# mikhaildubov/AST-text-analysis

Hardware: NVIDIA B200
Metric: keyphrase_x_doc_scores_per_sec (higher is better)
Workload: dtype f64

## Files before the change

### ast-text-analysis_b200/csrc/capi.cu

```cuda
#include <algorithm>
#include <array>
#include <chrono>
#include <cstdio>
#include <cstdlib>
#include <cstring>
#include <exception>
#include <map>
#include <memory>
#include <mutex>
#include <string>

#include "../../include/east_b200.h"
#include "sa_build.h"
#include "kp_prep.h"

namespace east {

thread_local int64_t g_launches = 0;
thread_local int g_time_kernels = 0;
thread_local double g_next_bytes = 0.0;

struct KernelStat { int64_t launches = 0; double ms = 0.0; double bytes = 0.0; };
struct PendingLaunch { std::string name; cudaEvent_t a, b; double bytes; };
static thread_local std::map<std::string, KernelStat> g_kstats;
// ... 474 lines not shown
    idx->next = take32((size_t)n);
    idx->ann = take32((size_t)n);

    if (text8_dev && !chunks) {
        DevBuf<uint32_t> bad(1, s);
        EAST_CUDA(cudaMemsetAsync(bad.p, 0, sizeof(uint32_t), s));
        expand_text8(text8_dev, idx->d_doc_off, idx->d_doc_m, n_docs, idx->text, bad.p, s);
        uint32_t h_bad = 0;
        EAST_CUDA(cudaMemcpyAsync(&h_bad, bad.p, sizeof(uint32_t), cudaMemcpyDeviceToHost, s));
        EAST_CUDA(cudaStreamSynchronize(s));
        if (h_bad) throw Error(EAST_ERR_INVALID, "one-byte text: a document does not hold exactly doc_m string ends (0xFF) or does not end with one");
    }
    idx->build_timer.reset(new StageTimer(s));
    StageTimer &tm = *idx->build_timer;
    const bool overlap = get_option("sync_build", 0) == 0;
    {
        SaInput in;
        in.text = idx->text; in.doc_off = idx->d_doc_off; in.doc_m = idx->d_doc_m;
        in.n = n; in.n_docs = n_docs; in.m_total = idx->m_total;
        in.key_chars = (int)get_option("key_chars", 0);
        in.force_general = (int)get_option("force_general", 0);
        in.rs_variant = (int)get_option("rs_variant", 0);
        in.doc_off_host = idx->doc_off.data();
        in.sort_batch_elems = get_option("sort_batch_elems", 0);
        in.local_group_sort = get_option("doubling_radix", 0) ? 0 : 1;
        in.segmented_sort = get_option("global_sort", 0) ? 0 : 1;
        in.doc_sort = (get_option("no_doc_sort", 0) || in.key_chars || in.rs_variant || in.sort_batch_elems ||
                       !in.segmented_sort || !in.local_group_sort) ? 0 : 1;
        in.want_bkt3 = get_option("no_bkt3", 0) ? 0 : 1;
        in.light_scan = get_option("no_light_scan", 0) ? 0 : 1;
        { const int64_t smp = get_option("alphabet_sample", (int64_t)1 << 21); in.alphabet_sample = smp < 0 ? 0 : smp; }
        in.alphabet_guess = get_option("no_alphabet_guess", 0) ? 0 : 1;
        in.fused_encode = get_option("no_fused_encode", 0) ? 0 : 1;
        if (!get_option("no_suffix_keys", 0)) {
            idx->sk = (uint32_t *)take32((size_t)n);
            in.sk = idx->sk;
        }
        if (!get_option("no_fused_tables", 0)) {
            in.lcp = idx->lcp; in.up = idx->up; in.down = idx->down; in.next = idx->next; in.ann = idx->ann;
        }
        in.arena = idx->arena.base ? &idx->arena : nullptr;
        in.helper_stream = aux_stream(device);
        if (!get_option("no_prep_stream", 0)) in.prep_stream = prep_stream(device);
        if (hook && hook->fn) {
            in.run_begin = hook->begin; in.run_hook = hook->fn; in.run_ctx = hook->ctx; in.scan_queued = hook->scan_queued;
            if (hook->building) *hook->building = idx.get();
        }
        if (chunks && text8_dev) {
            if (!in.doc_sort || !in.fused_encode) throw Error(EAST_ERR_INVALID, "internal: the one-byte pipelined build needs the per-document kernel");
            in.text8 = text8_dev;
        }
        if (chunks && in.doc_sort) {
            in.n_chunks = (int)chunks->ready.size();
            in.chunk_doc = chunks->doc.data();
            in.chunk_ready = chunks->ready.data();
        } else if (chunks) {
            for (auto e : chunks->ready) EAST_CUDA(cudaStreamWaitEvent(s, e, 0));
        }
        SaOutput so;
        so.sa = idx->sa;
        build_suffix_array(in, so, tm, s);
        idx->pipelined = so.pipelined; idx->pipeline_miss = so.pipeline_miss; idx->alphabet_miss = so.alphabet_miss; idx->alphabet_guessed = so.alphabet_guessed;
        idx->rounds = so.rounds; idx->fast_path = so.fast_path; idx->key_chars = so.key_chars;
        idx->key_bits = so.key_bits; idx->active_after_round0 = so.active_after_round0;
        idx->doc_sorted = so.doc_sorted; idx->doc_sort_overflow = so.doc_sort_overflow;
        idx->t8 = so.t8.p; so.t8.p = nullptr;
// ... 1216 lines not shown
```

### ast-text-analysis_b200/csrc/doc_sort.cu

```cuda
#include <cstdlib>
#include "sa_build.h"
#include "score_walk.cuh"

namespace east {

constexpr int DS_THREADS = 1024;
constexpr int DS_WARPS = DS_THREADS / 32;
constexpr int DS_GROUP = 128;
constexpr int DS_GWARPS = DS_GROUP / 32;
constexpr int DS_NGROUPS = DS_THREADS / DS_GROUP;
constexpr int DS_REFINE_MAX = 4096;
constexpr int DS_SUB_BINS = 1024;
constexpr int DS_GRP_BYTES = DS_REFINE_MAX * 2 + DS_SUB_BINS * 4;
constexpr int DS_SCR_BYTES = DS_NGROUPS * DS_GRP_BYTES;
constexpr int DS_WARP_MAX = 1024;
constexpr int DS_WARP_BYTES = DS_WARP_MAX * 2 + 128 * 4;
constexpr int DS_LIST_CAP = 2048;
constexpr int DS_WIN_BYTES = 64 * 8 + 64 * 4;
constexpr int DS_INF = 0x7fffffff;
static_assert(DS_WARPS * DS_WARP_BYTES <= DS_SCR_BYTES && DS_WARPS * DS_WIN_BYTES <= DS_SCR_BYTES, "scratch");
static_assert(8 * DocScore::MAX_GROUPS <= DS_SCR_BYTES, "phase 9 keeps the groups' maxima in shared memory");

struct DocSortParams {
    const uint8_t *t8;
    const uint32_t *text;
    const int32_t *doc_off;
    const int32_t *doc_m;
    int32_t *sa;
    uint32_t *bkt;
    uint32_t *bkt3;
    uint32_t *overflow;
    int b, G, S2;
    uint32_t term;
    int text_cap;
    int bits_words;
    int doc_begin;
    unsigned long long *phase_clk;
    int32_t *lcp, *up, *down, *next, *ann;
    uint32_t *sk;
    DocScore score;
    const uint8_t *code_table;
    uint8_t *t8_out;
    uint32_t *miss;
    int64_t text_len;
    const uint8_t *text8;
    uint32_t *text_out;
    int fill_early;
};

__device__ __forceinline__ uint64_t ds_lds8(const uint8_t *base, int o) {
    const uint32_t *q = reinterpret_cast<const uint32_t *>(base + (o & ~3));
    const uint32_t sh = (uint32_t)(o & 3) * 8u;
    const uint32_t w0 = q[0], w1 = q[1], w2 = q[2];
    return ((uint64_t)__funnelshift_r(w1, w2, sh) << 32) | __funnelshift_r(w0, w1, sh);
}
__device__ __forceinline__ uint32_t ds_lds4(const uint8_t *base, int o) {
    const uint32_t *q = reinterpret_cast<const uint32_t *>(base + (o & ~3));
    return __funnelshift_r(q[0], q[1], (uint32_t)(o & 3) * 8u);
}

__device__ __forceinline__ uint32_t ds_zero4(uint32_t v) {
    return ~(((v & 0x7f7f7f7fu) + 0x7f7f7f7fu) | v | 0x7f7f7f7fu);
}

__device__ __forceinline__ uint64_t ds_haszero(uint64_t v) {
    return (v - 0x0101010101010101ull) & ~v & 0x8080808080808080ull;
}

__device__ __forceinline__ uint32_t ds_id_from_word(uint32_t w, uint32_t term4, int b, int nsym) {
    const uint32_t z = ds_zero4(w ^ term4) & (0xffffffffu >> (8 * (4 - nsym)));
    if (z) w &= 0xffffffffu >> (8 * (3 - ((__ffs(z) - 1) >> 3)));
    const uint32_t s0 = w & 0xffu, s1 = (w >> 8) & 0xffu, s2 = (w >> 16) & 0xffu, s3 = w >> 24;
    switch (nsym) {
        case 1: return s0;
        case 2: return (s0 << b) | s1;
        case 3: return (((s0 << b) | s1) << b) | s2;
        default: return (((((s0 << b) | s1) << b) | s2) << b) | s3;
    }
}

// ... 14 lines not shown
__device__ __forceinline__ Ids8 ds_bucket8(const uint8_t *s_raw, int o, uint64_t term8, int b, int nsym) {
    Ids8 r;
    if (nsym <= 4) {
        const uint64_t x0 = ds_lds8(s_raw, o), x1 = ds_lds8(s_raw, o + 8);
        const uint32_t W[4] = {(uint32_t)x0, (uint32_t)(x0 >> 32), (uint32_t)x1, (uint32_t)(x1 >> 32)};
#pragma unroll
        for (int j = 0; j < 8; ++j)
            r.id[j] = ds_id_from_word(__funnelshift_r(W[j >> 2], W[(j >> 2) + 1], (uint32_t)(j & 3) * 8u), (uint32_t)term8, b, nsym);
    } else {
#pragma unroll
        for (int j = 0; j < 8; ++j) r.id[j] = ds_bucket(s_raw, o + j, term8, b, nsym);
    }
    return r;
}

__device__ __forceinline__ bool ds_id_has_term(uint32_t id, int nsym, int b, uint32_t term) {
    const uint32_t mask = (1u << b) - 1u;
    bool t = false;
    for (int g = 0; g < nsym; ++g) t = t || (((id >> (g * b)) & mask) == term);
    return t;
}

__device__ __forceinline__ uint64_t ds_key8(const uint8_t *s_raw, int o, uint64_t term8, int G) {
    const uint64_t x0 = ds_lds8(s_raw, o), x1 = ds_lds8(s_raw, o + 8);
    if (ds_haszero(x0 ^ term8) & ((1ull << (8 * G)) - 1ull)) return 0ull;
    uint64_t y = (x0 >> (8 * G)) | (x1 << (64 - 8 * G));
    const uint64_t z = ds_haszero(y ^ term8);
    if (z) {
        const int k = (__ffsll((long long)z) - 1) >> 3;
        if (k < 7) y &= (1ull << (8 * (k + 1))) - 1ull;
    }
    const uint32_t hi = __byte_perm((uint32_t)y, 0u, 0x0123), lo = __byte_perm((uint32_t)(y >> 32), 0u, 0x0123);
    return ((uint64_t)hi << 32) | lo;
}

__device__ __forceinline__ bool ds_deep_less(const uint8_t *s_raw, int oi, int oj, int from, uint64_t term8) {
    int o = from;
    while (true) {
        const uint64_t x = ds_lds8(s_raw, oi + o), y = ds_lds8(s_raw, oj + o);
        const uint64_t stop = (x ^ y) | ds_haszero(x ^ term8);
        if (stop) {
            const int sh = (__ffsll((long long)stop) - 1) & ~7;
            const uint32_t bx = (uint32_t)(x >> sh) & 0xffu, by = (uint32_t)(y >> sh) & 0xffu;
            if (bx != by) return bx < by;
            return oi < oj;
        }
        o += 8;
    }
}

__device__ __forceinline__ void ds_group_sync(int id) {
    asm volatile("bar.sync %0, %1;" ::"r"(id), "r"(DS_GROUP) : "memory");
}


struct DocCtx {
    const uint8_t *s_raw;
    int shift;
    uint64_t term8;
    uint32_t term;
    int b, S2;
    int32_t base;
    int32_t *sa_doc;
    uint32_t *s_bits;
    uint32_t *overflow;
};

__device__ __forceinline__ void ds_rank_by_position(const DocCtx &c, const uint16_t *pos, int start, int size, int t, int nthr) {
    const uint32_t *p2 = reinterpret_cast<const uint32_t *>(pos);
    for (int e = t; e < size; e += nthr) {
        const uint32_t pe = pos[e];
        int below = 0;
        for (int q = 0; q < (size >> 1); ++q) {
            const uint32_t v = p2[q];
            below += ((v & 0xffffu) < pe ? 1 : 0) + ((v >> 16) < pe ? 1 : 0);
        }
        if ((size & 1) && pos[size - 1] < pe) ++below;
        c.sa_doc[start + below] = c.base + (int32_t)pe;
    }
}

// ... 624 lines not shown
        uint8_t *gscr = reinterpret_cast<uint8_t *>(s_scr) + g * DS_GRP_BYTES;
        uint8_t *wscr = reinterpret_cast<uint8_t *>(s_scr) + warp * DS_WARP_BYTES;
        int cur = 0;
        while (true) {
            const int cnt = min((int)s_nlist[cur], DS_LIST_CAP);
            __syncthreads();
            if (cnt == 0) { if (tid == 0) s_work = 0; __syncthreads(); break; }
            if (tid == 0) { s_nlist[cur ^ 1] = 0; s_work = 0; }
            __syncthreads();
            uint2 *list = cur ? s_list1 : s_list0, *next = cur ? s_list0 : s_list1;
            bool any_big = false;
            while (true) {
                int e = 0;
                if (lane == 0) e = (int)atomicAdd(&s_work, 1u);
                e = __shfl_sync(0xffffffffu, e, 0);
                if (e >= cnt) break;
                const uint2 entry = list[e];
                if ((entry.x >> 16) > (uint32_t)DS_WARP_MAX) { any_big = true; continue; }
                ds_refine_warp(c, entry, lane, wscr, next, &s_nlist[cur ^ 1]);
            }
            if (__syncthreads_or(any_big ? 1 : 0)) {
                for (int e = g; e < cnt; e += DS_NGROUPS) {
                    const uint2 entry = list[e];
                    if ((entry.x >> 16) <= (uint32_t)DS_WARP_MAX) continue;
                    ds_refine(c, entry, g, gt, gscr, s_gmin, s_gw, next, &s_nlist[cur ^ 1]);
                }
                __syncthreads();
            }
            cur ^= 1;
        }
    }
    DS_STAMP(4);

    {
        uint64_t *wkeys = reinterpret_cast<uint64_t *>(reinterpret_cast<uint8_t *>(s_scr) + warp * DS_WIN_BYTES);
        uint32_t *wpos = reinterpret_cast<uint32_t *>(wkeys + 64);
        const int nwin = (n + 31) >> 5;
        while (true) {
            int w = 0;
            if (lane == 0) w = (int)atomicAdd(&s_work, 1u);
            w = __shfl_sync(0xffffffffu, w, 0);
            if (w >= nwin) break;
            uint32_t word = s_bits[w];
            const bool last_win = w == (n >> 5);
            if (last_win) word &= (1u << (n & 31)) - 1u;
            if (word == 0u) continue;
            const int r0 = 32 * w + (__ffs(word) - 1);
            int r1 = n;
            if (!last_win) {
                int ww = w + 1;
                uint32_t x;
                while ((x = s_bits[ww]) == 0u) ++ww;
                r1 = 32 * ww + (__ffs(x) - 1);
            }
            const int last_start = 32 * w + (31 - __clz(word));
            int nseg = __popc(word);
            if (r1 - last_start > 32) { r1 = last_start; --nseg; }
            const int len = r1 - r0;
            if (len <= nseg) continue;
            uint32_t seg[2];
            const int nslots = len > 32 ? 2 : 1;
#pragma unroll
            for (int s = 0; s < 2; ++s) {
                const int x = lane + 32 * s;
                seg[s] = 0;
                if (s < nslots && x < len) {
                    const int r = r0 + x;
                    const int li = sa_doc[r] - base;
                    const int wp = r - 32 * w;
                    const uint32_t le = (wp < 32) ? (word & (0xffffffffu >> (31 - wp))) : word;
                    const int sb = 32 * w + (31 - __clz(le)) - r0;
                    const uint32_t gt = (wp < 31) ? (word & (0xfffffffeu << wp)) : 0u;
                    int se = gt ? (32 * w + (__ffs(gt) - 1) - r0) : len;
                    if (se > len) se = len;
                    if (se - sb > 1) {
                        wkeys[x] = ds_key8(s_raw, shift + li, term8, G);
                        seg[s] = (uint32_t)sb | ((uint32_t)se << 8);
                    }
                    wpos[x] = (uint32_t)li;
                }
            }
            __syncwarp();
#pragma unroll
            for (int s = 0; s < 2; ++s) {
                const int x = lane + 32 * s;
                if (s < nslots && seg[s] != 0u) {
                    const int q0 = (int)(seg[s] & 0xffu), q1 = (int)(seg[s] >> 8);
                    const uint64_t key = wkeys[x];
                    const uint32_t li = wpos[x];
                    int below = 0;
                    const uint32_t last = (uint32_t)key & 0xffu;
                    const bool by_pos = last == 0u || last == p.term;
                    uint32_t ties = 0;
#pragma unroll 4
                    for (int q = q0; q < q1; ++q) {
                        const uint64_t kq = wkeys[q];
                        below += (kq < key) ? 1 : 0;
                        ties |= (kq == key ? 1u : 0u) << (q - q0);
                    }
                    ties &= ~(1u << (x - q0));
                    while (ties) {
                        const uint32_t pq = wpos[q0 + __ffs(ties) - 1];
                        ties &= ties - 1u;
                        const bool less = by_pos ? (pq < li) : ds_deep_less(s_raw, shift + (int)pq, shift + (int)li, G + 8, term8);
                        below += less ? 1 : 0;
                    }
                    seg[s] = (uint32_t)(q0 + below) | 0x100u;
                }
            }
            __syncwarp();
#pragma unroll
            for (int s = 0; s < 2; ++s) {
                const int x = lane + 32 * s;
                if (s < nslots && seg[s] != 0u) sa_doc[r0 + (int)(seg[s] & 0xffu)] = base + (int32_t)wpos[x];
            }
            __syncwarp();
        }
    }
    DS_STAMP(5);
    if (p.lcp == nullptr) {
        if (p.sk) {
            __syncthreads();
            for (int r = tid; r < n; r += DS_THREADS) p.sk[base + r] = ds_lds4(s_raw, shift + (sa_doc[r] - base) + 2);
        }
        ds_score_document<GROUPS>(p, ds_smem, p.text_cap + DS_SCR_BYTES + 4 * p.bits_words + 2 * (int)sizeof(uint2) * DS_LIST_CAP, doc, base, n, tid);
        return;
    }

    __syncthreads();
    uint16_t *s_lcp = reinterpret_cast<uint16_t *>(s_scr);
    __shared__ int s_pyr_off[4], s_pyr_size[4], s_pyr_levels;
    if (tid == 0) {
        int off = 0, sz = n, levels = 1;
        s_pyr_off[0] = 0; s_pyr_size[0] = n;
        for (int k = 1; k < 4; ++k) {
            off += (sz + 1) & ~1;
            sz = (sz + 31) >> 5;
            s_pyr_off[k] = off; s_pyr_size[k] = sz;
            levels = k + 1;
            if (sz <= 1) break;
        }
        s_pyr_levels = levels;
    }
    __syncthreads();
    if (p.fill_early) {
        int32_t *const up_doc = p.up + base, *const down_doc = p.down + base, *const next_doc = p.next + base, *const ann_doc = p.ann + base;
        for (int r = tid; r < n; r += DS_THREADS) { up_doc[r] = 0; down_doc[r] = 0; next_doc[r] = 0; ann_doc[r] = 0; }
    }
    SPyr M;
    M.lcp = s_lcp; M.off = s_pyr_off; M.size_ = s_pyr_size; M.levels = s_pyr_levels;
    uint16_t *s_lv1 = s_lcp + s_pyr_off[1];
// ... 157 lines not shown
    if (S2 > 7) S2 = 7;
    plan.b = b; plan.G = G; plan.S2 = S2;
    plan.text_cap = (max_doc_n + 15 + 48 + 16 + 15) & ~15;
    plan.bits_words = ((max_doc_n >> 5) + 3 + 1) & ~1;
    const size_t after_text = DS_SCR_BYTES + sizeof(uint32_t) * (size_t)plan.bits_words + 2 * sizeof(uint2) * (size_t)DS_LIST_CAP;
    plan.smem = (size_t)plan.text_cap + after_text;
    size_t need = 0;
    for (int sz = max_doc_n, k = 0; k < 4; ++k) { need += 2 * (((size_t)sz + 1) & ~(size_t)1); if (sz <= 1) break; sz = (sz + 31) >> 5; }
    plan.tables_fit = need <= after_text ? 1 : 0;
    return plan.smem <= (size_t)220 * 1024;
}

void doc_sort_launch(const DocSortPlan &plan, const uint8_t *t8, const uint32_t *text, const int32_t *doc_off,
                     const int32_t *doc_m, int doc_begin, int n_docs,
                     int64_t n_total, uint32_t term, int32_t *sa, uint32_t *bkt, uint32_t *bkt3, uint32_t *overflow, cudaStream_t s,
                     unsigned long long *phase_clk, const DocSortTables *tables, uint32_t *sk, const DocScore *score,
                     const uint8_t *code_table, uint32_t *miss, int64_t text_len, const uint8_t *text8) {
    const bool groups = score && score->recs && bkt && score->group_off;
    ensure_dynamic_smem(groups ? (const void *)k_doc_suffix_sort_groups : (const void *)k_doc_suffix_sort, 220 * 1024);
    DocSortParams p;
    p.t8 = t8; p.text = text; p.doc_off = doc_off; p.doc_m = doc_m; p.sa = sa; p.bkt = bkt; p.bkt3 = (plan.G == 3) ? bkt3 : nullptr; p.overflow = overflow;
    p.b = plan.b; p.G = plan.G; p.S2 = plan.S2; p.term = term;
    p.text_cap = plan.text_cap; p.bits_words = plan.bits_words;
    p.phase_clk = phase_clk;
    p.doc_begin = doc_begin;
    p.sk = sk;
    if (score && score->recs && bkt) p.score = *score;
    if (p.score.recs && p.score.skip_suffix_keys) p.sk = nullptr;
    p.code_table = (code_table && miss) ? code_table : nullptr;
    p.t8_out = const_cast<uint8_t *>(t8); p.miss = miss; p.text_len = text_len;
    p.text8 = p.code_table ? text8 : nullptr; p.text_out = const_cast<uint32_t *>(text);
    static const bool fill_early = getenv("EAST_DOC_SORT_FILL_EARLY") != nullptr;
    p.fill_early = fill_early ? 1 : 0;
    p.lcp = p.up = p.down = p.next = p.ann = nullptr;
    if (tables && plan.tables_fit) { p.lcp = tables->lcp; p.up = tables->up; p.down = tables->down; p.next = tables->next; p.ann = tables->ann; }
    EAST_BYTES(((p.lcp ? 25.0 : 5.0) + (p.code_table ? (p.text8 ? 5.0 : 4.0) : 0.0)) * (double)n_total + (p.score.recs ? p.score.algorithmic_bytes : 0.0));
    if (groups) EAST_LAUNCH(k_doc_suffix_sort_groups, n_docs, DS_THREADS, plan.smem, s, p);
    else EAST_LAUNCH(k_doc_suffix_sort, n_docs, DS_THREADS, plan.smem, s, p);
}

}
```

### ast-text-analysis_b200/csrc/sa_build.cu

```cuda
#include <cstdio>
#include <cstdlib>
#include <algorithm>
#include "radix_sort.cuh"
#include "sa_build.h"

namespace east {

template <int THREADS, int ITEMS, int MINB>
static void launch_onesweep(const uint64_t *kin, uint64_t *kout, const uint32_t *vin, uint32_t *vout, int32_t n,
                            int shift, const uint32_t *hist_excl, uint32_t *status, uint32_t *ticket,
                            cudaStream_t s) {
    using Cfg = RsCfg<THREADS, ITEMS>;
    auto kern = k_rs_onesweep<THREADS, ITEMS, MINB>;
    ensure_dynamic_smem((const void *)kern, Cfg::SMEM);
    const int tiles = rs_num_tiles(n, Cfg::TILE);
    EAST_BYTES(24.0 * n);
    if (g_time_kernels) ktime_begin("k_rs_onesweep", s);
    kern<<<tiles, THREADS, Cfg::SMEM, s>>>(kin, kout, vin, vout, n, shift, hist_excl, status, ticket,
                                           (const RsTileDesc *)nullptr, 0);
    if (g_time_kernels) ktime_end(s);
    ++g_launches;
    g_next_bytes = 0.0;
    cudaError_t e = cudaGetLastError();
    if (e != cudaSuccess) throw Error(-2, std::string("k_rs_onesweep launch: ") + cudaGetErrorString(e));
// ... 929 lines not shown

static bool build_pipelined(const SaInput &in, SaOutput &out, StageTimer &tm, cudaStream_t s, uint32_t &doc_sort_flags) {
    const int32_t n = in.n;
    const int D = in.n_docs;
    int32_t max_doc_n = 0;
    for (int d = 0; d < D; ++d) max_doc_n = std::max(max_doc_n, in.doc_off_host[d + 1] - in.doc_off_host[d]);
    tm.mark("alphabet");
    DevBuf<ScanResult> d_first(1, s);
    const int32_t n0 = in.doc_off_host[in.chunk_doc[1]];
    ScanResult first;
    PresentBits guess;
    const bool guessed = alphabet_guess_for(in, guess);
    if (guessed) {
        memset(&first, 0, sizeof(first));
        memcpy(first.present, guess.w, sizeof(guess.w));
    } else {
        EAST_CUDA(cudaMemsetAsync(d_first.p, 0, sizeof(ScanResult), s));
        EAST_CUDA(cudaStreamWaitEvent(s, in.chunk_ready[0], 0));
        if (in.text8) EAST_LAUNCH(k_alphabet8, grid_for(n0, 256 * 16, 4), 256, 0, s, in.text8, n0, d_first.p);
        else EAST_LAUNCH(k_alphabet, grid_for(n0, 256 * 4 * 4, 4), 256, 0, s, in.text, n0, d_first.p);
        EAST_CUDA(cudaMemcpyAsync(&first, d_first.p, sizeof(ScanResult), cudaMemcpyDeviceToHost, s));
        EAST_CUDA(cudaStreamSynchronize(s));
        host_debug_mark("scan back");
    }
    uint32_t *present = first.present;
    uint32_t extra[4] = {0u, 0u, 0u, 0u};
    complete_symbol_classes(present, extra);
    int sigma = 0;
    std::vector<uint8_t> table(EAST_TERM_BASE, 0);
    for (uint32_t c = 0; c < EAST_TERM_BASE; ++c)
        if (present[c >> 5] & (1u << (c & 31))) { ++sigma; table[c] = (uint8_t)(sigma & 0xff); }
    DocSortPlan plan;
    const bool eligible = sigma <= 253 && doc_sort_plan(sigma, max_doc_n, plan);
    const uint32_t term = (uint32_t)sigma + 1;

    DevBuf<uint8_t> t8;
    DevBuf<uint32_t> flags(2, s);
    if (eligible) {
        tm.mark("doc_sort");
        DevBuf<uint8_t> d_table(EAST_TERM_BASE, s);
        t8 = take<uint8_t>(in, (size_t)n + 128, s);
        uint32_t *end0 = nullptr, *end1 = nullptr;
        if (((size_t)D << (2 * plan.b)) <= (size_t)2 * n + 4096) {
            const size_t entries = ((size_t)D << (2 * plan.b)) + 1;
            out.bkt = take<uint32_t>(in, entries, s);
            end0 = out.bkt.p + entries - 1;
            out.sym_bits = plan.b;
            if (in.want_bkt3 && plan.G == 3 && ((size_t)D << (3 * plan.b)) * sizeof(uint32_t) <= ((size_t)8 << 30)) {
                const size_t e3 = ((size_t)D << (3 * plan.b)) + 1;
                out.bkt3 = take<uint32_t>(in, e3, s);
                end1 = out.bkt3.p + e3 - 1;
            }
        }
        {
            PresentBits bits;
            memcpy(bits.w, present, sizeof(bits.w));
            EAST_LAUNCH(k_doc_sort_prologue, 1, 128, 0, s, guessed ? (const ScanResult *)nullptr : d_first.p, bits,
                        make_uint4(extra[0], extra[1], extra[2], extra[3]), d_table.p, flags.p, end0, end1, (uint32_t)n);
            if (guessed) EAST_CUDA(cudaStreamWaitEvent(s, in.chunk_ready[0], 0));
        }
        DocSortTables tables{in.lcp, in.up, in.down, in.next, in.ann};
        const bool fuse = in.lcp != nullptr && plan.tables_fit;
        cudaStream_t lanes[2] = {s, in.helper_stream ? in.helper_stream : s};
        cudaStream_t prep = (in.prep_stream && lanes[1] != s && !in.fused_encode) ? in.prep_stream : nullptr;
        cudaEvent_t ready_to_sort = nullptr, helper_done = nullptr;
        if (lanes[1] != s) {
// ... 136 lines not shown
    bool fast = !scan.bad && (sampled || scan.n_term == (uint32_t)in.m_total) && sigma <= 253 && !in.force_general;
    out.fast_path = fast ? 1 : 0;
    out.sigma = sigma;

    const int dbits = bits_for((uint64_t)(D > 0 ? D - 1 : 0));
    KeyParams kp;
    if (fast) {
        kp.b = bits_for((uint64_t)sigma + 1);
        kp.term = (uint32_t)sigma + 1;
    } else {
        kp.b = bits_for((uint64_t)scan.max_code + 1);
        kp.term = 0xffffffffu;
    }
    if (dbits + kp.b > 64) throw Error(-5, "document count x alphabet does not fit a 64-bit sort key");
    int kc = (64 - dbits) / kp.b;
    if (kc > KG_HALO) kc = KG_HALO;
    {
        const bool seg_like = fast && in.segmented_sort && (int64_t)n / D >= 2 * RS_SEG_TILE && in.sort_batch_elems == 0;
        const int extra = seg_like ? 0 : dbits;
        if (kc > 8 && rs_num_passes(extra + (kc - 1) * kp.b) < rs_num_passes(extra + kc * kp.b)) --kc;
    }
    if (in.key_chars > 0 && in.key_chars < kc) kc = in.key_chars;
    kp.kc = kc;
    const int key_bits = dbits + kc * kp.b;
    kp.passes = rs_num_passes(key_bits);
    out.key_chars = kc;
    out.key_bits = key_bits;

    tm.mark("encode");
    DevBuf<uint8_t> t8, d_table;
    size_t arena_after_t8 = arena_mark;
    DocSortPlan doc_plan;
    const bool try_doc_sort = fast && allow_doc_sort && doc_sort_plan(sigma, max_doc_n, doc_plan);
    bool coded = false;
    auto encode_all = [&]() {
        EAST_BYTES(5.0 * n);
        EAST_LAUNCH(k_encode_text, grid_for(n, 256 * 4 * 4, 4), 256, 0, s, in.text, 0, n, d_table.p,
                    (uint8_t)kp.term, t8.p, (uint32_t *)nullptr);
        coded = true;
    };
    const bool table_in_prologue = try_doc_sort && in.fused_encode;
    if (fast) {
        d_table = DevBuf<uint8_t>(EAST_TERM_BASE, s);
        if (!table_in_prologue) {
            if (guessed) {
                PresentBits bits;
                memcpy(bits.w, scan.present, sizeof(bits.w));
                EAST_LAUNCH(k_set_present, 1, 128, 0, s, d_scan.p, bits);
            }
            EAST_LAUNCH(k_code_table, 1, 128, 0, s, d_scan.p, d_table.p, make_uint4(extra[0], extra[1], extra[2], extra[3]));
        }
        t8 = take<uint8_t>(in, (size_t)n + 128, s);
        arena_after_t8 = in.arena ? in.arena->used : 0;
        if (!table_in_prologue) encode_all();
    }
    out.code_table = table;
    out.term_code = fast ? (int)kp.term : 0;

    if (sampled && !try_doc_sort) {
        if (guessed) g_alphabet_guess.valid = false;
        t8.release();
        if (in.arena) in.arena->used = arena_mark;
        SaInput again = in;
        again.alphabet_sample = 0;
        build_suffix_array(again, out, tm, s);
        return;
// ... 22 lines not shown
                EAST_LAUNCH(k_doc_sort_prologue, 1, 128, 0, s, guessed ? (const ScanResult *)nullptr : d_scan.p, bits,
                            make_uint4(extra[0], extra[1], extra[2], extra[3]), d_table.p, flag.p, end0, end1, (uint32_t)n);
            } else {
                EAST_CUDA(cudaMemsetAsync(flag.p, 0, 2 * sizeof(uint32_t), s));
                if (end0) EAST_LAUNCH(k_store_u32, 1, 1, 0, s, end0, (uint32_t)n);
                if (end1) EAST_LAUNCH(k_store_u32, 1, 1, 0, s, end1, (uint32_t)n);
            }
            static const bool profile = getenv("EAST_DOC_SORT_PROFILE") != nullptr;
            DevBuf<unsigned long long> clk;
            if (profile) {
                clk = DevBuf<unsigned long long>(16, s);
                EAST_CUDA(cudaMemsetAsync(clk.p, 0, 16 * sizeof(unsigned long long), s));
            }
            DocSortTables tables{in.lcp, in.up, in.down, in.next, in.ann};
            const bool fuse = in.lcp != nullptr && plan.tables_fit;
            const bool hooks = out.bkt.p != nullptr;
            const RunReady run{0, D, s, t8.p, out.bkt.p, out.bkt3.p, out.sym_bits, &table, 0};
            DocScore score;
            if (hooks && in.run_begin) in.run_begin(in.run_ctx, run, score);
            doc_sort_launch(plan, t8.p, in.text, in.doc_off, in.doc_m, 0, D, n, kp.term, out.sa, out.bkt.p, out.bkt3.p, flag.p, s, clk.p,
                            fuse ? &tables : nullptr, in.sk, &score, coded ? nullptr : d_table.p, flag.p + 1, n);
            uint32_t h_flag[2] = {0u, 0u};
            EAST_CUDA(cudaMemcpyAsync(h_flag, flag.p, sizeof(h_flag), cudaMemcpyDeviceToHost, s));
            EAST_CUDA(cudaStreamSynchronize(s));
            const uint32_t overflow = h_flag[0];
            const bool missed = sampled && h_flag[1] != 0u;
            if (profile) {
                unsigned long long h[16];
                EAST_CUDA(cudaMemcpy(h, clk.p, sizeof(h), cudaMemcpyDeviceToHost));
                static const char *names[10] = {"load", "hist", "scan", "scatter", "refine", "windows", "lcp", "stack_walk", "beyond_chunk", "score"};
                fprintf(stderr, "[east] doc_sort phases, kilo-cycles per document:");
                for (int k = 0; k < 10; ++k) fprintf(stderr, " %s %.1f", names[k], (double)h[k] / D / 1e3);
                fprintf(stderr, "\n");
            }
            if (missed) {
                if (guessed) g_alphabet_guess.valid = false;
                out.bkt = DevBuf<uint32_t>();
                out.bkt3 = DevBuf<uint32_t>();
                out.sym_bits = 0;
                t8.release();
                if (in.arena) in.arena->used = arena_mark;
                SaInput again = in;
                again.alphabet_sample = 0;
                build_suffix_array(again, out, tm, s);
                out.alphabet_miss = 1;
                out.alphabet_guessed = guessed ? 1 : 0;
                return;
            }
            if (!overflow) {
                alphabet_guess_keep(scan.present);
                if (hooks && in.run_hook) in.run_hook(in.run_ctx, run, score.recs != nullptr ? 1 : 0);
                if (score.recs && score.skip_suffix_keys) out.sk_skipped = 1;
                out.doc_sorted = 1;
                out.tables_done = fuse ? 1 : 0;
                out.sk_done = in.sk ? 1 : 0;
                out.rounds = 1;
                out.key_chars = plan.G + 8;
                out.key_bits = plan.b * plan.G + 64;
                out.t8 = std::move(t8);
                return;
            }
            doc_sort_flags = overflow;
            out.doc_sort_overflow = (overflow & 1u) ? 1 : 0;
            out.bkt = DevBuf<uint32_t>();
            out.bkt3 = DevBuf<uint32_t>();
            out.sym_bits = 0;
// ... 174 lines not shown
```

### ast-text-analysis_b200/csrc/sa_build.h

```cpp
#pragma once
#include "common.cuh"

namespace east {

struct SufRec;
struct DocScore {
    const SufRec *recs = nullptr;
    int32_t n_uniq = 0;
    const uint8_t *q8 = nullptr;
    const uint32_t *kp = nullptr;
    double *tmp = nullptr;
    int normalized = 0;
    const int32_t *kp_off = nullptr;
    const int32_t *uniq_of = nullptr;
    int32_t K = 0;
    double *out = nullptr;
    const int32_t *group_off = nullptr;
    int32_t G = 0;
    static constexpr int32_t MAX_GROUPS = 12288;
    static constexpr int MAX_PEERS = 15;
    double *peer_out[MAX_PEERS] = {};
    int32_t n_peers = 0;
    double algorithmic_bytes = 0.0;
    int skip_suffix_keys = 0;
// ... 2 lines not shown
struct RunReady {
    int32_t doc_begin, doc_count;
    cudaStream_t stream;
    const uint8_t *t8;
    const uint32_t *bkt, *bkt3;
    int sym_bits;
    const std::vector<uint8_t> *code_table;
    int speculative;
};

struct SaInput {
    const uint32_t *text;
    const uint8_t *text8 = nullptr;
    const int32_t *doc_off;
    const int32_t *doc_m;
    int32_t n;
    int32_t n_docs;
    int64_t m_total;
    int key_chars;
    int force_general;
    int rs_variant = 0;
    const int32_t *doc_off_host = nullptr;
    int segmented_sort = 1;
    int local_group_sort = 1;
    int64_t sort_batch_elems = 0;
    int doc_sort = 1;
    int32_t *lcp = nullptr, *up = nullptr, *down = nullptr, *next = nullptr, *ann = nullptr;
    uint32_t *sk = nullptr;
    int light_scan = 1;
    int64_t alphabet_sample = 0;
    int alphabet_guess = 0;
    int want_bkt3 = 1;
    int fused_encode = 1;
    int n_chunks = 0;
    const int32_t *chunk_doc = nullptr;
    const cudaEvent_t *chunk_ready = nullptr;
    cudaStream_t helper_stream = nullptr;
    cudaStream_t prep_stream = nullptr;
    void (*run_begin)(void *ctx, const RunReady &run, DocScore &score) = nullptr;
    void (*run_hook)(void *ctx, const RunReady &run, int in_kernel) = nullptr;
    void *run_ctx = nullptr;
    void (*scan_queued)(void *ctx) = nullptr;
    Arena *arena = nullptr;
};

struct SaOutput {
    int32_t *sa;
    DevBuf<uint8_t> t8;
    DevBuf<uint32_t> bkt;
    DevBuf<uint32_t> bkt3;
    std::vector<uint8_t> code_table;
    int sym_bits = 0;
    int term_code = 0;
    int fast_path = 0;
    int sigma = 0;
    int key_chars = 0;
    int key_bits = 0;
    int rounds = 0;
    uint32_t active_after_round0 = 0;
    int segmented = 0;
    int radix_fallback_rounds = 0;
    int doc_sorted = 0;
    int doc_sort_overflow = 0;
    int tables_done = 0;
    int sk_done = 0;
    int sk_skipped = 0;
    int pipelined = 0;
    int pipeline_miss = 0;
    int alphabet_guessed = 0;
    int alphabet_miss = 0;
};

void build_suffix_array(const SaInput &in, SaOutput &out, StageTimer &tm, cudaStream_t s);
void expand_text8(const uint8_t *text8, const int32_t *doc_off, const int32_t *doc_m, int n_docs, uint32_t *text, uint32_t *bad,
                  cudaStream_t s);

struct DocSortPlan {
    int b = 0, G = 0, S2 = 0;
    int text_cap = 0, bits_words = 0;
    size_t smem = 0;
    int tables_fit = 0;
};
struct DocSortTables { int32_t *lcp, *up, *down, *next, *ann; };
bool doc_sort_plan(int sigma, int32_t max_doc_n, DocSortPlan &plan);
void doc_sort_launch(const DocSortPlan &plan, const uint8_t *t8, const uint32_t *text, const int32_t *doc_off,
                     const int32_t *doc_m, int doc_begin, int n_docs,
                     int64_t n_total , uint32_t term, int32_t *sa, uint32_t *bkt, uint32_t *bkt3, uint32_t *overflow, cudaStream_t s,
                     unsigned long long *phase_clk = nullptr ,
                     const DocSortTables *tables = nullptr ,
                     uint32_t *sk = nullptr ,
                     const DocScore *score = nullptr ,
                     const uint8_t *code_table = nullptr ,
                     uint32_t *miss = nullptr, int64_t text_len = 0 ,
                     const uint8_t *text8 = nullptr );

void tokenize_texts(const uint8_t *raw_dev, const int64_t *raw_off_dev, int32_t n_texts, int32_t *sizes_dev, cudaStream_t s);
void tokenize_emit(const uint8_t *raw_dev, const int64_t *raw_off_dev, int32_t n_texts, const int64_t *doc_off_dev, uint32_t *text_dev,
                   cudaStream_t s);

void build_lcp_tables(const uint32_t *text, const uint8_t *t8 , int term_code, const int32_t *sa, const int32_t *doc_off, const int32_t *doc_m,
                      int n_docs, int32_t n, int32_t *lcp, int32_t *up, int32_t *down, int32_t *next,
                      int32_t *ann, StageTimer &tm, cudaStream_t s, int child_variant = 0);

bool alphabet_guess_code_table(uint8_t *table );
void alphabet_guess_forget();

struct SufRec {
    uint64_t q8_first;
    int32_t sidx;
    uint16_t len;
    uint8_t generic;
    uint8_t pad;
};
struct ScoreInput {
// ... 39 lines not shown
```

Measured before the change: 300.2 million.

## Pack small-bucket windows per warp and compare bit-packed wider suffix keys

Makes a new default path for sorting the small buckets inside the per-document suffix sort. Warps claim 128-rank spans through an atomic counter and pack consecutive small buckets into 32-lane passes. Each suffix gets a 64-bit key of up to S symbols, bit-packed at b bits per symbol rather than one byte per symbol, which should cut the costly deep tie-break comparisons. The old byte-key window path stays behind a window_bytekeys option, and profiling counters for passes, trips and deep compares are added when phase clocks are on. The risk is extra key-packing arithmetic and a different load balance across warps.

```diff
diff --git a/ast-text-analysis_b200/csrc/capi.cu b/ast-text-analysis_b200/csrc/capi.cu
--- a/ast-text-analysis_b200/csrc/capi.cu
+++ b/ast-text-analysis_b200/csrc/capi.cu
@@ -530,6 +530,7 @@
         { const int64_t smp = get_option("alphabet_sample", (int64_t)1 << 21); in.alphabet_sample = smp < 0 ? 0 : smp; }
         in.alphabet_guess = get_option("no_alphabet_guess", 0) ? 0 : 1;
         in.fused_encode = get_option("no_fused_encode", 0) ? 0 : 1;
+        in.window_bytekeys = get_option("window_bytekeys", 0) ? 1 : 0;
         if (!get_option("no_suffix_keys", 0)) {
             idx->sk = (uint32_t *)take32((size_t)n);
             in.sk = idx->sk;
diff --git a/ast-text-analysis_b200/csrc/doc_sort.cu b/ast-text-analysis_b200/csrc/doc_sort.cu
--- a/ast-text-analysis_b200/csrc/doc_sort.cu
+++ b/ast-text-analysis_b200/csrc/doc_sort.cu
@@ -17,6 +17,7 @@
 constexpr int DS_WARP_BYTES = DS_WARP_MAX * 2 + 128 * 4;
 constexpr int DS_LIST_CAP = 2048;
 constexpr int DS_WIN_BYTES = 64 * 8 + 64 * 4;
+constexpr int DS_SPAN_WORDS = 4;
 constexpr int DS_INF = 0x7fffffff;
 static_assert(DS_WARPS * DS_WARP_BYTES <= DS_SCR_BYTES && DS_WARPS * DS_WIN_BYTES <= DS_SCR_BYTES, "scratch");
 static_assert(8 * DocScore::MAX_GROUPS <= DS_SCR_BYTES, "phase 9 keeps the groups' maxima in shared memory");
@@ -46,6 +47,7 @@
     const uint8_t *text8;
     uint32_t *text_out;
     int fill_early;
+    int window_bytekeys;
 };
 
 __device__ __forceinline__ uint64_t ds_lds8(const uint8_t *base, int o) {
@@ -126,6 +128,34 @@
     }
     const uint32_t hi = __byte_perm((uint32_t)y, 0u, 0x0123), lo = __byte_perm((uint32_t)(y >> 32), 0u, 0x0123);
     return ((uint64_t)hi << 32) | lo;
+}
+
+__device__ __forceinline__ uint32_t ds_pack4(uint32_t w, int b) {
+    const uint32_t t = ((w & 0x00ff00ffu) << b) | ((w >> 8) & 0x00ff00ffu);
+    return ((t & 0xffffu) << (2 * b)) | (t >> 16);
+}
+__device__ __forceinline__ uint64_t ds_pack8(uint64_t y, int b) {
+    return ((uint64_t)ds_pack4((uint32_t)y, b) << (4 * b)) | ds_pack4((uint32_t)(y >> 32), b);
+}
+
+__device__ __forceinline__ uint64_t ds_keyp(const uint8_t *s_raw, int o, uint64_t term8, int G, int b, int S) {
+    const uint64_t x0 = ds_lds8(s_raw, o), x1 = ds_lds8(s_raw, o + 8);
+    if (ds_haszero(x0 ^ term8) & ((1ull << (8 * G)) - 1ull)) return 0ull;
+    uint64_t y0 = (x0 >> (8 * G)) | (x1 << (64 - 8 * G));
+    uint64_t y1 = x1 >> (8 * G);
+    const uint64_t z0 = ds_haszero(y0 ^ term8);
+    if (z0) {
+        const int k = (__ffsll((long long)z0) - 1) >> 3;
+        if (k < 7) y0 &= (1ull << (8 * (k + 1))) - 1ull;
+        y1 = 0ull;
+    } else {
+        const uint64_t z1 = ds_haszero(y1 ^ term8);
+        if (z1) {
+            const int k = (__ffsll((long long)z1) - 1) >> 3;
+            if (k < 7) y1 &= (1ull << (8 * (k + 1))) - 1ull;
+        }
+    }
+    return (ds_pack8(y0, b) << (b * (S - 8))) | (ds_pack8(y1, b) >> (b * (16 - S)));
 }
 
 __device__ __forceinline__ bool ds_deep_less(const uint8_t *s_raw, int oi, int oj, int from, uint64_t term8) {
@@ -141,6 +171,12 @@
         }
         o += 8;
     }
+}
+
+__device__ __forceinline__ void ds_count_pass(unsigned long long *prof, int lane, uint32_t trips, uint32_t deep) {
+    trips = __reduce_max_sync(0xffffffffu, trips);
+    deep = __reduce_add_sync(0xffffffffu, deep);
+    if (lane == 0) { prof[0] += 1ull; prof[1] += trips; prof[2] += deep; }
 }
 
 __device__ __forceinline__ void ds_group_sync(int id) {
@@ -831,6 +867,93 @@
     }
     DS_STAMP(4);
 
+    __shared__ unsigned long long s_prof[DS_WARPS][4];
+    if (p.phase_clk && lane < 4) s_prof[warp][lane] = 0ull;
+    __syncwarp();
+    if (!p.window_bytekeys) {
+        uint64_t *wkeys = reinterpret_cast<uint64_t *>(reinterpret_cast<uint8_t *>(s_scr) + warp * DS_WIN_BYTES);
+        uint32_t *wpos = reinterpret_cast<uint32_t *>(wkeys + 32);
+        const int S = min(64 / b, 16 - G);
+        const uint32_t last_mask = (1u << b) - 1u;
+        const int nspan = (n + 32 * DS_SPAN_WORDS - 1) / (32 * DS_SPAN_WORDS);
+        while (true) {
+            int sp = 0;
+            if (lane == 0) sp = (int)atomicAdd(&s_work, 1u);
+            sp = __shfl_sync(0xffffffffu, sp, 0);
+            if (sp >= nspan) break;
+            const int w0 = sp * DS_SPAN_WORDS;
+            const int span_end = min(n, 32 * (w0 + DS_SPAN_WORDS));
+            uint32_t word = (lane < DS_SPAN_WORDS && w0 + lane <= (n >> 5)) ? s_bits[w0 + lane] : 0u;
+            const uint32_t nz = __ballot_sync(0xffffffffu, word != 0u);
+            if (nz == 0u) continue;
+            word = __shfl_sync(0xffffffffu, word, __ffs(nz) - 1);
+            int r = 32 * (w0 + __ffs(nz) - 1) + (__ffs(word) - 1);
+            while (r < span_end) {
+                int rr = r + 1 + lane;
+                uint32_t M = __ballot_sync(0xffffffffu, rr <= n && ((s_bits[rr >> 5] >> (rr & 31)) & 1u));
+                if (M & 1u) { r += (M == 0xffffffffu) ? 32 : __ffs(~M) - 1; continue; }
+                if (M == 0u) {
+                    for (r += 33; r < span_end; r += 32) {
+                        rr = r + lane;
+                        M = __ballot_sync(0xffffffffu, rr <= n && ((s_bits[rr >> 5] >> (rr & 31)) & 1u));
+                        if (M) { r += __ffs(M) - 1; break; }
+                    }
+                    continue;
+                }
+                const int J = span_end - (r + 1);
+                uint32_t ends = M;
+                if (J < 32) { const uint32_t hi = M & (0xffffffffu << J); ends = (M & ~(0xffffffffu << J)) | (hi & (0u - hi)); }
+                const int len = 32 - __clz(ends);
+                long long t_setup = 0;
+                if (p.phase_clk && lane == 0) t_setup = clock64();
+                uint32_t seg = 0;
+                uint32_t li = 0;
+                if (lane < len) {
+                    li = (uint32_t)(sa_doc[r + lane] - base);
+                    const uint32_t before = M & ((1u << lane) - 1u);
+                    const int sb = before ? 32 - __clz(before) : 0;
+                    const int se = lane + __ffs(M >> lane);
+                    if (se - sb > 1) {
+                        wkeys[lane] = ds_keyp(s_raw, shift + (int)li, term8, G, b, S);
+                        seg = (uint32_t)sb | ((uint32_t)se << 8);
+                    }
+                    wpos[lane] = li;
+                }
+                __syncwarp();
+                if (p.phase_clk && lane == 0) s_prof[warp][3] += (unsigned long long)(clock64() - t_setup);
+                int deep = 0, trips = 0;
+                if (seg != 0u) {
+                    const int q0 = (int)(seg & 0xffu), q1 = (int)(seg >> 8);
+                    trips = q1 - q0;
+                    const uint64_t key = wkeys[lane];
+                    int below = 0;
+                    const uint32_t last = (uint32_t)key & last_mask;
+                    const bool by_pos = last == 0u || last == p.term;
+                    uint32_t ties = 0;
+#pragma unroll 4
+                    for (int q = q0; q < q1; ++q) {
+                        const uint64_t kq = wkeys[q];
+                        below += (kq < key) ? 1 : 0;
+                        ties |= (kq == key ? 1u : 0u) << (q - q0);
+                    }
+                    ties &= ~(1u << (lane - q0));
+                    if (!by_pos) deep = __popc(ties);
+                    while (ties) {
+                        const uint32_t pq = wpos[q0 + __ffs(ties) - 1];
+                        ties &= ties - 1u;
+                        const bool less = by_pos ? (pq < li) : ds_deep_less(s_raw, shift + (int)pq, shift + (int)li, G + S, term8);
+                        below += less ? 1 : 0;
+                    }
+                    seg = (uint32_t)(q0 + below) | 0x100u;
+                }
+                if (p.phase_clk) ds_count_pass(s_prof[warp], lane, (uint32_t)trips, (uint32_t)deep);
+                __syncwarp();
+                if (seg != 0u) sa_doc[r + (int)(seg & 0xffu)] = base + (int32_t)li;
+                __syncwarp();
+                r += len;
+            }
+        }
+    } else
     {
         uint64_t *wkeys = reinterpret_cast<uint64_t *>(reinterpret_cast<uint8_t *>(s_scr) + warp * DS_WIN_BYTES);
         uint32_t *wpos = reinterpret_cast<uint32_t *>(wkeys + 64);
@@ -859,6 +982,8 @@
             if (len <= nseg) continue;
             uint32_t seg[2];
             const int nslots = len > 32 ? 2 : 1;
+            long long t_setup = 0;
+            if (p.phase_clk && lane == 0) t_setup = clock64();
 #pragma unroll
             for (int s = 0; s < 2; ++s) {
                 const int x = lane + 32 * s;
@@ -880,11 +1005,14 @@
                 }
             }
             __syncwarp();
+            if (p.phase_clk && lane == 0) s_prof[warp][3] += (unsigned long long)(clock64() - t_setup);
 #pragma unroll
             for (int s = 0; s < 2; ++s) {
                 const int x = lane + 32 * s;
+                int deep = 0, trips = 0;
                 if (s < nslots && seg[s] != 0u) {
                     const int q0 = (int)(seg[s] & 0xffu), q1 = (int)(seg[s] >> 8);
+                    trips = q1 - q0;
                     const uint64_t key = wkeys[x];
                     const uint32_t li = wpos[x];
                     int below = 0;
@@ -898,6 +1026,7 @@
                         ties |= (kq == key ? 1u : 0u) << (q - q0);
                     }
                     ties &= ~(1u << (x - q0));
+                    if (!by_pos) deep = __popc(ties);
                     while (ties) {
                         const uint32_t pq = wpos[q0 + __ffs(ties) - 1];
                         ties &= ties - 1u;
@@ -906,6 +1035,7 @@
                     }
                     seg[s] = (uint32_t)(q0 + below) | 0x100u;
                 }
+                if (p.phase_clk && s < nslots) ds_count_pass(s_prof[warp], lane, (uint32_t)trips, (uint32_t)deep);
             }
             __syncwarp();
 #pragma unroll
@@ -916,6 +1046,7 @@
             __syncwarp();
         }
     }
+    if (p.phase_clk && lane < 4) atomicAdd(&p.phase_clk[10 + lane], s_prof[warp][lane]);
     DS_STAMP(5);
     if (p.lcp == nullptr) {
         if (p.sk) {
@@ -1139,6 +1270,7 @@
     p.text8 = p.code_table ? text8 : nullptr; p.text_out = const_cast<uint32_t *>(text);
     static const bool fill_early = getenv("EAST_DOC_SORT_FILL_EARLY") != nullptr;
     p.fill_early = fill_early ? 1 : 0;
+    p.window_bytekeys = plan.window_bytekeys;
     p.lcp = p.up = p.down = p.next = p.ann = nullptr;
     if (tables && plan.tables_fit) { p.lcp = tables->lcp; p.up = tables->up; p.down = tables->down; p.next = tables->next; p.ann = tables->ann; }
     EAST_BYTES(((p.lcp ? 25.0 : 5.0) + (p.code_table ? (p.text8 ? 5.0 : 4.0) : 0.0)) * (double)n_total + (p.score.recs ? p.score.algorithmic_bytes : 0.0));
diff --git a/ast-text-analysis_b200/csrc/sa_build.cu b/ast-text-analysis_b200/csrc/sa_build.cu
--- a/ast-text-analysis_b200/csrc/sa_build.cu
+++ b/ast-text-analysis_b200/csrc/sa_build.cu
@@ -985,6 +985,7 @@
         if (present[c >> 5] & (1u << (c & 31))) { ++sigma; table[c] = (uint8_t)(sigma & 0xff); }
     DocSortPlan plan;
     const bool eligible = sigma <= 253 && doc_sort_plan(sigma, max_doc_n, plan);
+    plan.window_bytekeys = in.window_bytekeys;
     const uint32_t term = (uint32_t)sigma + 1;
 
     DevBuf<uint8_t> t8;
@@ -1187,6 +1188,7 @@
     size_t arena_after_t8 = arena_mark;
     DocSortPlan doc_plan;
     const bool try_doc_sort = fast && allow_doc_sort && doc_sort_plan(sigma, max_doc_n, doc_plan);
+    doc_plan.window_bytekeys = in.window_bytekeys;
     bool coded = false;
     auto encode_all = [&]() {
         EAST_BYTES(5.0 * n);
@@ -1275,6 +1277,8 @@
                 fprintf(stderr, "[east] doc_sort phases, kilo-cycles per document:");
                 for (int k = 0; k < 10; ++k) fprintf(stderr, " %s %.1f", names[k], (double)h[k] / D / 1e3);
                 fprintf(stderr, "\n");
+                fprintf(stderr, "[east] doc_sort windows per document: passes %.1f trips %.1f deep %.1f setup_kcycles %.1f\n",
+                        (double)h[10] / D, (double)h[11] / D, (double)h[12] / D, (double)h[13] / D / 1e3);
             }
             if (missed) {
                 if (guessed) g_alphabet_guess.valid = false;
diff --git a/ast-text-analysis_b200/csrc/sa_build.h b/ast-text-analysis_b200/csrc/sa_build.h
--- a/ast-text-analysis_b200/csrc/sa_build.h
+++ b/ast-text-analysis_b200/csrc/sa_build.h
@@ -58,6 +58,7 @@
     int alphabet_guess = 0;
     int want_bkt3 = 1;
     int fused_encode = 1;
+    int window_bytekeys = 0;
     int n_chunks = 0;
     const int32_t *chunk_doc = nullptr;
     const cudaEvent_t *chunk_ready = nullptr;
@@ -106,6 +107,7 @@
     int text_cap = 0, bits_words = 0;
     size_t smem = 0;
     int tables_fit = 0;
+    int window_bytekeys = 0;
 };
 struct DocSortTables { int32_t *lcp, *up, *down, *next, *ann; };
 bool doc_sort_plan(int sigma, int32_t max_doc_n, DocSortPlan &plan);
diff --git a/profiles/window_stats.py b/profiles/window_stats.py
--- /dev/null
+++ b/profiles/window_stats.py
@@ -0,0 +1,151 @@
+#!/usr/bin/env python3
+import argparse
+import os
+import sys
+
+ROOT = os.path.dirname(os.path.dirname(os.path.abspath(__file__)))
+sys.path.insert(0, os.path.join(ROOT, "ast-text-analysis_b200")); sys.path.insert(0, ROOT)
+import numpy as np
+
+import synth
+from oracle import oracle
+
+
+def plan(sigma):
+    b = (sigma + 1).bit_length()
+    G = min(7, 15 // b)
+    return b, G, max(1, min(7, 10 // b)), min(64 // b, 16 - G)
+
+
+def cut_windows(codes, term, width):
+    n = len(codes)
+    pad = np.concatenate([codes, np.full(width, term, dtype=np.int64)])
+    win = np.stack([pad[i:i + n] for i in range(width)], axis=1)
+    seen = np.cumsum(win == term, axis=1)
+    after = (seen - (win == term)) > 0
+    win[after] = 0
+    return win
+
+
+def small_buckets(codes, term, sa, b, G, S2):
+    n = len(sa)
+    pad = np.concatenate([codes, np.full(64, term, dtype=np.int64)])
+    ids = cut_windows(codes, term, G)[sa]
+    starts = np.concatenate([[0], np.nonzero(np.any(ids[1:] != ids[:-1], axis=1))[0] + 1, [n]])
+    work = [(int(s), int(e), G, bool((ids[s] == term).any())) for s, e in zip(starts[:-1], starts[1:])]
+    out, single, all_starts = [], 0, []
+    while work:
+        s, e, depth, terminal = work.pop()
+        size = e - s
+        if size <= 32 or terminal:
+            all_starts.append(s)
+        if size == 1:
+            single += 1
+            continue
+        if size <= 32:
+            out.append((s, size, depth))
+            continue
+        if terminal:
+            continue
+        pos = sa[s:e]
+        d = depth
+        while True:
+            col = pad[pos + d]
+            if (col != col[0]).any() or col[0] == term:
+                break
+            d += 1
+        if (pad[pos + d] == term).all():
+            all_starts.append(s)
+            continue
+        width = S2 if size > 1024 else 1
+        win = np.stack([pad[pos + d + k] for k in range(width)], axis=1)
+        seen = np.cumsum(win == term, axis=1)
+        win[(seen - (win == term)) > 0] = 0
+        cuts = np.concatenate([[0], np.nonzero(np.any(win[1:] != win[:-1], axis=1))[0] + 1, [size]])
+        for a, z in zip(cuts[:-1], cuts[1:]):
+            work.append((s + int(a), s + int(z), d + width, bool((win[a] == term).any())))
+    out.sort()
+    return out, single, sorted(all_starts) + [n]
+
+
+def windows(n, buckets, starts):
+    starts = np.asarray(starts)
+    passes = trips = 0
+    for w in range((n + 31) >> 5):
+        inside = starts[(starts >= 32 * w) & (starts < min(n, 32 * w + 32))]
+        if len(inside) == 0:
+            continue
+        r0, last = int(inside[0]), int(inside[-1])
+        r1 = int(starts[np.searchsorted(starts, 32 * w + 32)]) if 32 * w + 32 < n else n
+        nseg = len(inside)
+        if r1 - last > 32:
+            r1, nseg = last, nseg - 1
+        if r1 - r0 <= nseg:
+            continue
+        for slot in range(2 if r1 - r0 > 32 else 1):
+            lo, hi = r0 + 32 * slot, min(r1, r0 + 32 * slot + 32)
+            sizes = [size for s, size, _ in buckets if s < hi and s + size > lo and 32 * w <= s < 32 * w + 32]
+            passes += 1
+            trips += max(sizes) if sizes else 0
+    return passes, trips
+
+
+def packs(n, buckets, span=128):
+    passes = trips = 0
+    i = 0
+    while i < len(buckets):
+        s0 = buckets[i][0]
+        end_span = (s0 // span + 1) * span
+        first, top = s0, 0
+        while i < len(buckets) and buckets[i][0] < end_span and buckets[i][0] + buckets[i][1] - first <= 32:
+            top = max(top, buckets[i][1])
+            i += 1
+        passes += 1
+        trips += top
+    return passes, trips
+
+
+def tie_pairs(lcp, buckets, G, S):
+    pairs = 0
+    for s, size, _ in buckets:
+        for i in range(s, s + size):
+            run = 1 << 30
+            for j in range(i + 1, s + size):
+                run = min(run, int(lcp[j]))
+                if run < G + S:
+                    break
+                pairs += 2
+    return pairs
+
+
+def main():
+    ap = argparse.ArgumentParser()
+    ap.add_argument("--docs", type=int, default=2)
+    ap.add_argument("--doc-bytes", type=int, default=50000)
+    ap.add_argument("--seed", type=int, default=1)
+    a = ap.parse_args()
+    oracle.build()
+    packed, ms, _ = synth.packed_collection(a.docs, a.doc_bytes, first_seed=a.seed)
+    for d, (text, m) in enumerate(zip(packed, ms)):
+        text = np.asarray(text, dtype=np.int64)
+        letters = np.unique(text[text < 0x0A00])
+        sigma = len(letters)
+        term = sigma + 1
+        codes = np.where(text < 0x0A00, np.searchsorted(letters, text) + 1, term).astype(np.int64)
+        b, G, S2, S = plan(sigma)
+        o = oracle.OracleEASA(text=packed[d], m=m)
+        sa, lcp = np.asarray(o.suftab, dtype=np.int64), np.asarray(o.lcptab, dtype=np.int64)
+        n = len(sa)
+        buckets, single, starts = small_buckets(codes, term, sa, b, G, S2)
+        sizes = np.array([size for _, size, _ in buckets])
+        wp, wt = windows(n, buckets, starts)
+        pp, pt = packs(n, buckets)
+        print("doc %d: n %d sigma %d b %d G %d S %d | small buckets %d holding %d (mean %.1f, max %d), singletons %d"
+              % (d, n, sigma, b, G, S, len(buckets), sizes.sum(), sizes.mean(), sizes.max(), single))
+        print("  windows of 32 ranks: passes %d loop trips %d | packs: passes %d loop trips %d"
+              % (wp, wt, pp, pt))
+        print("  deep comparisons: S = 8 %d | S = %d %d" % (tie_pairs(lcp, buckets, G, 8), S, tie_pairs(lcp, buckets, G, S)))
+
+
+if __name__ == "__main__":
+    main()
```

New measurement: 305.2 million, median of 6. 1.7% higher.
